# SowpatiLab/ribbit

Hardware: AMD Instinct MI355X
Metric: Gbases/s scanned (m=2..100) (higher is better)
Workload: dtype u32 bit planes

## Files before the change

ribbit_amd/csrc/kernels.hip:

```cpp
#include <hip/hip_runtime.h>

#include <algorithm>
#include <climits>
#include <type_traits>

#include "kernels.h"

namespace rb {

__device__ __forceinline__ uint32_t funnel(uint32_t hi, uint32_t lo, uint32_t sh) {
    return __builtin_amdgcn_alignbit(hi, lo, sh);
}

template <unsigned TT>
__device__ __forceinline__ uint32_t bitop3(uint32_t a, uint32_t b, uint32_t c) {
    return __builtin_amdgcn_bitop3_b32(a, b, c, TT);
}

__global__ __launch_bounds__(256) void pack_kernel(const uint8_t *__restrict__ ascii, int64_t length,
                                                   uint32_t *__restrict__ hi, uint32_t *__restrict__ lo,
                                                   uint32_t *__restrict__ brk, int64_t total_words,
                                                   uint32_t *__restrict__ zero_words, int n_zero) {
    const int64_t t = (int64_t)blockIdx.x * blockDim.x + threadIdx.x;
    if (blockIdx.x == 0)
// ... 43 lines not shown
            h |= __builtin_amdgcn_udot4(b2 & ok, weights, 0u, false) << (4 * i);
            l |= __builtin_amdgcn_udot4(lo1 & ok, weights, 0u, false) << (4 * i);
            b |= __builtin_amdgcn_udot4(bad, weights, 0u, false) << (4 * i);
        }
        if (left < 32) b |= 0xffffffffu << (uint32_t)left;
    }
    hi[t] = h; lo[t] = l; brk[t] = b;
}

void launch_pack(const uint8_t *dev_ascii, int64_t length, uint32_t *hi, uint32_t *lo, uint32_t *brk,
                 int64_t total_words, uint32_t *zero_words, int n_zero, hipStream_t stream) {
    const int threads = 256;
    const int64_t blocks = (total_words + threads - 1) / threads;
    hipLaunchKernelGGL(pack_kernel, dim3((unsigned)blocks), dim3(threads), 0, stream, dev_ascii, length, hi, lo, brk,
                       total_words, zero_words, n_zero);
}

constexpr int EV_STAGE = 256;

__device__ __forceinline__ int wave_inclusive_scan(int v) {
    v += __builtin_amdgcn_update_dpp(0, v, 0x111, 0xf, 0xf, true);
    v += __builtin_amdgcn_update_dpp(0, v, 0x112, 0xf, 0xf, true);
    v += __builtin_amdgcn_update_dpp(0, v, 0x114, 0xf, 0xf, true);
    v += __builtin_amdgcn_update_dpp(0, v, 0x118, 0xf, 0xf, true);
    v += __builtin_amdgcn_update_dpp(0, v, 0x142, 0xa, 0xf, false);
    v += __builtin_amdgcn_update_dpp(0, v, 0x143, 0xc, 0xf, false);
    return v;
}

struct EventSink {
    uint64_t *events;
    uint32_t *counters;
    uint32_t region_cap;
    uint32_t shard;
};

__device__ __forceinline__ void sink_flush(const EventSink &sk, volatile uint64_t *stage, int &staged, int lane) {
    if (staged == 0) return;
    uint32_t base = 0;
    if (lane == 0) base = atomicAdd(&sk.counters[sk.shard * EV_COUNTER_STRIDE], (uint32_t)staged);
    base = (uint32_t)__builtin_amdgcn_readfirstlane((int)base);
    uint64_t *dst = sk.events + (size_t)sk.shard * sk.region_cap;
    for (int i = lane; i < staged; i += 64) {
        const uint32_t idx = base + (uint32_t)i;
        if (idx < sk.region_cap) dst[idx] = stage[i];
    }
    __builtin_amdgcn_wave_barrier();
    staged = 0;
}

template <typename EndKind>
__device__ __forceinline__ void stage_events(const uint32_t (&S)[WORDS_PER_LANE], const uint32_t (&E)[WORDS_PER_LANE],
                                             uint32_t word0, uint32_t mlen, const EventSink &sink,
                                             volatile uint64_t *stage, int &staged, int lane, EndKind end_kind) {
    uint32_t Sv[WORDS_PER_LANE], Ev[WORDS_PER_LANE];
#pragma unroll
    for (int k = 0; k < WORDS_PER_LANE; k++) {
        Sv[k] = S[k]; Ev[k] = E[k];
        asm volatile("" : "+v"(Sv[k]), "+v"(Ev[k]));
    }
    int cnt = 0;
#pragma unroll
    for (int k = 0; k < WORDS_PER_LANE; k++) cnt += __popc(Sv[k]) + __popc(Ev[k]);
    const int incl = wave_inclusive_scan(cnt);
    const int total = __builtin_amdgcn_readlane(incl, 63);
    if (staged + total > EV_STAGE) sink_flush(sink, stage, staged, lane);
    const bool direct = total > EV_STAGE;
    uint32_t idx = (uint32_t)(incl - cnt);
    uint64_t *gdst = nullptr;
    if (direct) {
        uint32_t base = 0;
        if (lane == 0) base = atomicAdd(&sink.counters[sink.shard * EV_COUNTER_STRIDE], (uint32_t)total);
        idx += (uint32_t)__builtin_amdgcn_readfirstlane((int)base);
        gdst = sink.events + (size_t)sink.shard * sink.region_cap;
    } else {
        idx += (uint32_t)staged;
    }
#pragma unroll
    for (int k = 0; k < WORDS_PER_LANE; k++) {
        uint32_t both = Sv[k] | Ev[k];
        while (both) {
            const uint32_t b = (uint32_t)__builtin_ctz(both);
            both &= both - 1u;
            const uint32_t pos = ((word0 + (uint32_t)k) << 5) + b;
            const uint32_t kind = ((Sv[k] >> b) & 1u) ? (uint32_t)EV_START : end_kind(k, b, pos);
            const uint64_t e = ev_pack(pos, mlen, kind);
            if (direct) { if (idx < sink.region_cap) gdst[idx] = e; }
            else stage[idx] = e;
            idx++;
        }
    }
    if (!direct) staged += total;
    __builtin_amdgcn_wave_barrier();
}

constexpr int K = WORDS_PER_LANE;

#ifndef RB_COOP_MAX_LANES
#define RB_COOP_MAX_LANES 16
#endif
constexpr int COOP_SRC = 16;
struct CoopScratch { uint32_t w[COOP_SRC][20]; };

__device__ __forceinline__ void stage_events_coop(const uint32_t (&S)[WORDS_PER_LANE], const uint32_t (&E)[WORDS_PER_LANE], uint32_t word0, uint32_t mlen,
                                                  uint32_t brk_at, const uint32_t *s_brk, uint32_t length, CoopScratch &sc, const EventSink &sink,
                                                  volatile uint64_t *stage, int &staged, int lane) {
    uint32_t Sv[WORDS_PER_LANE], Ev[WORDS_PER_LANE];
#pragma unroll
    for (int k = 0; k < WORDS_PER_LANE; k++) {
        Sv[k] = S[k]; Ev[k] = E[k];
        asm volatile("" : "+v"(Sv[k]), "+v"(Ev[k]));
    }
    int cnt = 0;
#pragma unroll
    for (int k = 0; k < WORDS_PER_LANE; k++) cnt += __popc(Sv[k] | Ev[k]);
    const int incl = wave_inclusive_scan(cnt);
    const int total = __builtin_amdgcn_readlane(incl, 63);
    if (staged + total > EV_STAGE) sink_flush(sink, stage, staged, lane);
    const bool direct = total > EV_STAGE;
    uint32_t first = (uint32_t)(incl - cnt);
    uint64_t *gdst = nullptr;
    if (direct) {
        uint32_t base = 0;
        if (lane == 0) base = atomicAdd(&sink.counters[sink.shard * EV_COUNTER_STRIDE], (uint32_t)total);
        first += (uint32_t)__builtin_amdgcn_readfirstlane((int)base);
        gdst = sink.events + (size_t)sink.shard * sink.region_cap;
    } else {
        first += (uint32_t)staged;
    }
    unsigned long long todo = __ballot(cnt != 0);
    const int r = lane >> 2, j = lane & 3;
    do {
        const int rank = (int)__builtin_amdgcn_mbcnt_hi((uint32_t)(todo >> 32), __builtin_amdgcn_mbcnt_lo((uint32_t)todo, 0u));
        const bool mine = ((todo >> lane) & 1ull) != 0ull && rank < COOP_SRC;
        if (mine) {
            uint32_t *row = sc.w[rank];
#pragma unroll
            for (int k = 0; k < WORDS_PER_LANE; k++) { row[k] = Sv[k]; row[WORDS_PER_LANE + k] = Ev[k]; }
            row[16] = word0; row[17] = mlen; row[18] = brk_at; row[19] = first;
        }
        const unsigned long long handled = __ballot(mine);
        const int nsrc = __popcll(handled);
        todo &= ~handled;
        __builtin_amdgcn_wave_barrier();
        uint32_t s0 = 0, s1 = 0, e0 = 0, e1 = 0;
        if (r < nsrc) { s0 = sc.w[r][2 * j]; s1 = sc.w[r][2 * j + 1]; e0 = sc.w[r][WORDS_PER_LANE + 2 * j]; e1 = sc.w[r][WORDS_PER_LANE + 2 * j + 1]; }
        const int c = __popc(s0 | e0) + __popc(s1 | e1);
        const int q0 = __builtin_amdgcn_update_dpp(0, c, 0x00, 0xf, 0xf, true);
        const int q1 = __builtin_amdgcn_update_dpp(0, c, 0x55, 0xf, 0xf, true);
        const int q2 = __builtin_amdgcn_update_dpp(0, c, 0xaa, 0xf, 0xf, true);
        if (c != 0) {
            const uint32_t w0 = sc.w[r][16], ml = sc.w[r][17], bb = sc.w[r][18];
            uint32_t idx = sc.w[r][19] + (uint32_t)((j > 0 ? q0 : 0) + (j > 1 ? q1 : 0) + (j > 2 ? q2 : 0));
            auto expand = [&](uint32_t sw, uint32_t ew, uint32_t k) {
                uint32_t both = sw | ew;
                while (both) {
                    const uint32_t b = (uint32_t)__builtin_ctz(both);
                    both &= both - 1u;
                    const uint32_t pos = ((w0 + k) << 5) + b;
                    uint32_t kind = (uint32_t)EV_START;
                    if (!((sw >> b) & 1u))
                        kind = pos >= length ? (uint32_t)EV_END_EOS : (((s_brk[bb + k] >> b) & 1u) ? (uint32_t)EV_END_N : (uint32_t)EV_END_ZERO);
                    const uint64_t e = ev_pack(pos, ml, kind);
                    if (direct) { if (idx < sink.region_cap) gdst[idx] = e; }
                    else stage[idx] = e;
                    idx++;
                }
            };
            expand(s0, e0, 2u * (uint32_t)j);
            expand(s1, e1, 2u * (uint32_t)j + 1u);
        }
        __builtin_amdgcn_wave_barrier();
    } while (RB_COOP_MAX_LANES > COOP_SRC && todo != 0ull);
    if (!direct) staged += total;
}
__device__ __forceinline__ void group_filter(const uint32_t (&PASS)[K + 2], const uint32_t (&EVAL)[K + 2], int tj, uint32_t (&SV)[K + 1],
                                             uint32_t (&DR)[K]) {
    uint32_t J[K + 2], W[K + 2];
#pragma unroll
    for (int j = K + 1; j >= 1; j--) J[j] = PASS[j] | funnel(PASS[j], PASS[j - 1], 31);
    J[0] = PASS[0] | (PASS[0] << 1);
#pragma unroll
    for (int j = K + 1; j >= 1; j--) J[j] = J[j] | funnel(J[j], J[j - 1], 30);
    J[0] = J[0] | (J[0] << 2);
#pragma unroll
    for (int j = K + 1; j >= 1; j--) J[j] = J[j] | funnel(J[j], J[j - 1], 28);
    J[0] = J[0] | (J[0] << 4);
#pragma unroll
    for (int j = 0; j < K + 1; j++) J[j] = J[j] & funnel(J[j + 1], J[j], 1);
    J[K + 1] = J[K + 1] & (J[K + 1] >> 1);
#pragma unroll
    for (int j = 0; j < K + 1; j++) J[j] = J[j] & funnel(J[j + 1], J[j], 2);
    J[K + 1] = J[K + 1] & (J[K + 1] >> 2);
#pragma unroll
    for (int j = 0; j < K + 1; j++) J[j] = J[j] & funnel(J[j + 1], J[j], 4);
    J[K + 1] = J[K + 1] & (J[K + 1] >> 4);
#pragma unroll
    for (int j = 0; j < K + 2; j++) J[j] |= PASS[j];
#pragma unroll
    for (int j = 0; j < K + 2; j++) W[j] = J[j];
    {
        int span = 1;
#pragma unroll
        for (int step = 0; step < 4; step++) {
            const int sh = min(span, tj - span);
            if (sh > 0) {
#pragma unroll
                for (int j = 0; j < K + 1; j++) W[j] = W[j] & funnel(W[j + 1], W[j], (uint32_t)sh);
                W[K + 1] = W[K + 1] & (W[K + 1] >> sh);
                span += sh;
            }
        }
        span = 1;
#pragma unroll
        for (int step = 0; step < 4; step++) {
            const int sh = min(span, tj - span);
            if (sh > 0) {
#pragma unroll
                for (int j = K + 1; j >= 1; j--) W[j] = W[j] | funnel(W[j], W[j - 1], (uint32_t)(32 - sh));
                W[0] = W[0] | (W[0] << sh);
                span += sh;
            }
        }
    }
    auto special_ends = [&](int j) {
        const uint32_t jprev = j > 0 ? funnel(J[j], J[j - 1], 31) : (J[0] << 1);
        const uint32_t ev8 = j < K + 1 ? funnel(EVAL[j + 1], EVAL[j], 8) : (EVAL[K + 1] >> 8);
        const uint32_t g = ~J[j] & jprev & ~(EVAL[j] & ev8);
        return j == 0 ? 0u : (j == K + 1 ? (g & 0x0000ffffu) : g);
    };
    uint32_t special = 0;
#pragma unroll
    for (int j = 1; j < K + 2; j++) special |= special_ends(j);
    if (__ballot(special != 0) != 0ull) {
        uint32_t G[K + 2], JL[K + 2];
#pragma unroll
        for (int j = 0; j < K + 2; j++) { JL[j] = J[j]; G[j] = special_ends(j); }
#pragma unroll
        for (int j = 0; j < K + 1; j++) G[j] = funnel(G[j + 1], G[j], 1) & J[j];
        G[K + 1] = (G[K + 1] >> 1) & J[K + 1];
#pragma unroll
        for (int sh = 1; sh <= 8; sh <<= 1) {
#pragma unroll
            for (int j = 0; j < K + 1; j++) G[j] |= funnel(G[j + 1], G[j], (uint32_t)sh) & JL[j];
            G[K + 1] |= (G[K + 1] >> sh) & JL[K + 1];
#pragma unroll
            for (int j = 0; j < K + 1; j++) JL[j] = JL[j] & funnel(JL[j + 1], JL[j], (uint32_t)sh);
            JL[K + 1] = JL[K + 1] & (JL[K + 1] >> sh);
        }
#pragma unroll
        for (int j = 0; j < K + 1; j++) W[j] |= G[j];
    }
#pragma unroll
    for (int j = 0; j < K + 1; j++) SV[j] = W[j];
#pragma unroll
    for (int k = 0; k < K; k++) {
        const uint32_t jprev = funnel(J[k + 1], J[k], 31);
        const uint32_t svprev = funnel(W[k + 1], W[k], 31);
        DR[k] = ~J[k + 1] & jprev & ~svprev;
    }
}

constexpr int LDS_EXTRA = 40;

template <bool UNIFORM>
__device__ __forceinline__ uint32_t perfect_edges(const uint32_t (&Z)[K + 2], uint32_t t3, uint32_t t4, uint32_t t5,
                                                  uint32_t back, uint32_t (&SQ)[K], uint32_t (&EQ)[K]) {
    uint32_t D[K + 2];
#pragma unroll
    for (int j = 0; j < K + 1; j++) D[j] = Z[j] | funnel(Z[j + 1], Z[j], 1);
    D[K + 1] = Z[K + 1] | (Z[K + 1] >> 1);
#pragma unroll
    for (int j = 0; j < K + 1; j++) D[j] = D[j] | funnel(D[j + 1], D[j], 2);
    D[K + 1] = D[K + 1] | (D[K + 1] >> 2);
#pragma unroll
    for (int j = 0; j < K + 1; j++) D[j] = D[j] | funnel(D[j + 1], D[j], t3);
    D[K + 1] = D[K + 1] | (D[K + 1] >> t3);
#pragma unroll
    for (int j = 0; j < K + 1; j++) D[j] = D[j] | funnel(D[j + 1], D[j], t4);
    if (!UNIFORM || t5) {
        D[K + 1] = D[K + 1] | (D[K + 1] >> t4);
#pragma unroll
        for (int j = 0; j < K + 1; j++) D[j] = D[j] | funnel(D[j + 1], D[j], t5);
    }
    uint32_t any = 0;
#pragma unroll
    for (int k = 0; k < K; k++) {
        const int j = k + 1;
        const uint32_t prev_z = funnel(Z[j], Z[j - 1], 31);
        const uint32_t d_back = funnel(D[j], D[j - 1], back);
        SQ[k] = prev_z & ~D[j];
        EQ[k] = Z[j] & ~d_back;
        any = bitop3<0xFE>(SQ[k], EQ[k], any);
    }
    return any;
}

constexpr int CAND_CAP = 64;
#ifndef RB_CAND_DIRECT
#define RB_CAND_DIRECT 32
#endif
constexpr int CAND_DIRECT = RB_CAND_DIRECT;
struct CandQueue {
    uint32_t z[K + 2][CAND_CAP];
    uint32_t tag[CAND_CAP];
};

#ifndef RB_PERFECT_WAVES
#define RB_PERFECT_WAVES 4
#endif
__global__ __launch_bounds__(256) __attribute__((amdgpu_waves_per_eu(RB_PERFECT_WAVES, RB_PERFECT_WAVES))) void scan_perfect_kernel(DevicePlanes pl, PerfectLaunch pp, int motifs_per_block,
                                                           uint64_t *__restrict__ events,
                                                           uint32_t *__restrict__ counters) {
    __shared__ uint32_t s_hi[TILE_WORDS + LDS_EXTRA];
    __shared__ uint32_t s_lo[TILE_WORDS + LDS_EXTRA];
    __shared__ uint32_t s_brk[TILE_WORDS + 8];
    __shared__ uint64_t s_stage[4][EV_STAGE];
    __shared__ CandQueue s_cand[4];
    __shared__ CoopScratch s_coop[4];

    const int lane = threadIdx.x & 63;
    const int wave = __builtin_amdgcn_readfirstlane((int)(threadIdx.x >> 6));
    const int64_t tile_base = (int64_t)blockIdx.x * TILE_WORDS;

    const int bm_lo = pp.m_lo + (int)blockIdx.y * motifs_per_block;
    const int bm_hi = min(pp.m_hi, bm_lo + motifs_per_block - 1);
    const int q_hi = bm_hi >> 5;

    const int n_ext = TILE_WORDS + 4 + q_hi;
    for (int i = threadIdx.x; i < n_ext; i += 256) {
        s_hi[i] = pl.hi[tile_base - 1 + i];
        s_lo[i] = pl.lo[tile_base - 1 + i];
    }
    for (int i = threadIdx.x; i < TILE_WORDS + 2; i += 256) s_brk[i] = pl.brk[tile_base - 1 + i];
    __syncthreads();

    const int wm_lo = bm_lo + wave;
    const int wm_hi = bm_hi;
    if (wm_lo > wm_hi) return;

    const int lb = lane * K;
    uint32_t H[K + 2], Lo[K + 2], Bk[K + 2];
#pragma unroll
    for (int j = 0; j < K + 2; j++) { H[j] = s_hi[lb + j]; Lo[j] = s_lo[lb + j]; Bk[j] = s_brk[lb + j]; }

    uint32_t Hq[K + 3], Lq[K + 3];
    int cur_q = -1;
    const uint32_t length = (uint32_t)pl.length;
    const uint32_t word0 = (uint32_t)(tile_base + lb);

    EventSink sink;
    sink.events = events;
    sink.counters = counters;
    sink.region_cap = pp.ev_cap / EV_SHARDS;
    sink.shard = (blockIdx.x * 4u + (uint32_t)wave + blockIdx.y) % EV_SHARDS;
    volatile uint64_t *stage = s_stage[wave];
    int staged = 0;

    CandQueue &cq = s_cand[wave];
    int queued = 0;
    auto flush_candidates = [&]() {
        if (queued == 0) return;
        const bool live = lane < queued;
        const uint32_t tag = live ? cq.tag[lane] : 0u;
        const uint32_t src = tag & 0xffu, qm = tag >> 8;
        uint32_t Zq[K + 2];
#pragma unroll
        for (int j = 0; j < K + 2; j++) Zq[j] = live ? cq.z[j][lane] : 0xffffffffu;
        const int c1 = (qm <= 6u) ? 12 - (int)qm : (int)qm;
        const int sp = live ? min(c1, 32) : 32;
        const uint32_t t3 = (uint32_t)min(4, sp - 4);
        const uint32_t t4 = (uint32_t)min(8, sp - 4 - (int)t3);
        const uint32_t t5 = (uint32_t)(sp - 4) - t3 - t4;
        uint32_t SQ[K], EQ[K];
        uint32_t any = perfect_edges<false>(Zq, t3, t4, t5, 32u - (uint32_t)sp, SQ, EQ);
        if (!live) {
            any = 0;
#pragma unroll
            for (int k = 0; k < K; k++) { SQ[k] = 0; EQ[k] = 0; }
        }
#ifdef RB_ABLATE_STAGING
        const unsigned long long with_events = __ballot(any == 0xdeadbeefu);
#else
        const unsigned long long with_events = __ballot(any != 0);
#endif
        if (with_events != 0ull) {
            const uint32_t src_word0 = (uint32_t)tile_base + src * (uint32_t)K;
            if (__popcll(with_events) <= RB_COOP_MAX_LANES)
                stage_events_coop(SQ, EQ, src_word0, qm, src * (uint32_t)K + 1u, s_brk, length, s_coop[wave], sink, stage, staged, lane);
            else
                stage_events(SQ, EQ, src_word0, qm, sink, stage, staged, lane, [&](int k, uint32_t b, uint32_t pos) {
                    if (pos >= length) return (uint32_t)EV_END_EOS;
                    return ((s_brk[src * (uint32_t)K + (uint32_t)k + 1u] >> b) & 1u) ? (uint32_t)EV_END_N : (uint32_t)EV_END_ZERO;
                });
        }
        queued = 0;
        __builtin_amdgcn_wave_barrier();
    };

    for (int m = wm_lo; m <= wm_hi; m += 4) {
        const int q = m >> 5;
        const uint32_t r = (uint32_t)m & 31u;
        if (q != cur_q) {
            cur_q = q;
#pragma unroll
            for (int j = 0; j < K + 3; j++) { Hq[j] = s_hi[lb + j + q]; Lq[j] = s_lo[lb + j + q]; }
        }
        const int c1 = (m <= 6) ? 12 - m : m;
        const int sp = min(c1, 32);
        const uint32_t t3 = (uint32_t)min(4, sp - 4);
        const uint32_t t4 = (uint32_t)min(8, sp - 4 - (int)t3);
        const uint32_t t5 = (uint32_t)(sp - 4) - t3 - t4;

        uint32_t Z[K + 2];
#pragma unroll
        for (int j = 0; j < K + 2; j++) {
            const uint32_t hs = funnel(Hq[j + 1], Hq[j], r);
            const uint32_t ls = funnel(Lq[j + 1], Lq[j], r);
            Z[j] = bitop3<0xF6>(bitop3<0xBE>(H[j], hs, Bk[j]), Lo[j], ls);
        }
        if (sp >= 7) {
            bool cand;
            if (sp >= 31) {
                typedef unsigned short half2 __attribute__((ext_vector_type(2)));
                auto pk_min = [](uint32_t a, uint32_t b) {
                    const half2 m = __builtin_elementwise_min(__builtin_bit_cast(half2, a), __builtin_bit_cast(half2, b));
                    return __builtin_bit_cast(uint32_t, m);
                };
                uint32_t lowest = Z[0];
#pragma unroll
                for (int j = 1; j < K + 2; j++) lowest = pk_min(lowest, Z[j]);
                cand = (((lowest - 0x00010001u) & ~lowest) & 0x80008000u) != 0;
            } else {
                const uint32_t ones = sp >= 15 ? 0x01010101u : 0x11111111u;
                const uint32_t tops = sp >= 15 ? 0x80808080u : 0x88888888u;
                uint32_t hit = 0;
#pragma unroll
                for (int j = 0; j < K + 2; j++) hit = bitop3<0xBA>(Z[j] - ones, Z[j], hit);
                cand = (hit & tops) != 0;
            }
#ifdef RB_ABLATE_CHAIN
            const unsigned long long mask = __ballot(cand && Z[0] == 0xdeadbeefu);
#else
            const unsigned long long mask = __ballot(cand);
#endif
            if (mask == 0ull) continue;
            const int n = __popcll(mask);
            if (n <= CAND_DIRECT) {
                if (queued + n > CAND_CAP) flush_candidates();
                if (cand) {
                    const int slot = queued + (int)__builtin_amdgcn_mbcnt_hi((uint32_t)(mask >> 32), __builtin_amdgcn_mbcnt_lo((uint32_t)mask, 0u));
#pragma unroll
                    for (int j = 0; j < K + 2; j++) cq.z[j][slot] = Z[j];
                    cq.tag[slot] = (uint32_t)lane | ((uint32_t)m << 8);
                }
                queued += n;
                __builtin_amdgcn_wave_barrier();
                continue;
            }
        }
        uint32_t SQ[K], EQ[K];
        const uint32_t any = perfect_edges<true>(Z, t3, t4, t5, 32u - (uint32_t)sp, SQ, EQ);
#ifdef RB_ABLATE_STAGING
        const unsigned long long with_events = __ballot(any == 0xdeadbeefu);
#else
        const unsigned long long with_events = __ballot(any != 0);
#endif
        if (with_events != 0ull) {
            if (__popcll(with_events) <= RB_COOP_MAX_LANES)
                stage_events_coop(SQ, EQ, word0, (uint32_t)m, (uint32_t)lb + 1u, s_brk, length, s_coop[wave], sink, stage, staged, lane);
            else
                stage_events(SQ, EQ, word0, (uint32_t)m, sink, stage, staged, lane, [&](int k, uint32_t b, uint32_t pos) {
                    if (pos >= length) return (uint32_t)EV_END_EOS;
                    return ((Bk[k + 1] >> b) & 1u) ? (uint32_t)EV_END_N : (uint32_t)EV_END_ZERO;
                });
        }
    }
    flush_candidates();
    sink_flush(sink, stage, staged, lane);
}

static ScanSplit scan_split(const PerfectLaunch &pp, int nm, int64_t want_y, int max_y) {
    int motifs_per_block;
    if (pp.motifs_per_block > 0) {
        motifs_per_block = std::min(pp.motifs_per_block, nm);
    } else {
        const int gy = (int)(want_y < 1 ? 1 : (want_y > max_y ? max_y : want_y));
        motifs_per_block = (nm + gy - 1) / gy;
    }
    ScanSplit sp;
    sp.motifs_per_block = motifs_per_block;
    sp.grid_y = (nm + motifs_per_block - 1) / motifs_per_block;
    return sp;
}

ScanSplit launch_scan_perfect(const DevicePlanes &pl, const PerfectLaunch &pp, uint64_t *events, uint32_t *counters,
                              hipStream_t stream) {
    const int nm = pp.m_hi - pp.m_lo + 1;
    if (nm <= 0 || pl.ntiles <= 0) return {};
    const ScanSplit sp = scan_split(pp, nm, (2048 + pl.ntiles - 1) / pl.ntiles, (nm + 3) / 4);
    dim3 grid((unsigned)pl.ntiles, (unsigned)sp.grid_y);
    hipLaunchKernelGGL(scan_perfect_kernel, grid, dim3(256), 0, stream, pl, pp, sp.motifs_per_block, events, counters);
    return sp;
}

template <int ALLOWED>
__global__ __launch_bounds__(256) void scan_window_kernel(DevicePlanes pl, PerfectLaunch pp, int motifs_per_block,
                                                          uint64_t *__restrict__ events,
                                                          uint32_t *__restrict__ counters) {
    __shared__ uint32_t s_hi[TILE_WORDS + LDS_EXTRA];
    __shared__ uint32_t s_lo[TILE_WORDS + LDS_EXTRA];
    __shared__ uint32_t s_brk[TILE_WORDS + 8];
    __shared__ uint64_t s_stage[4][EV_STAGE];

    const int lane = threadIdx.x & 63;
    const int wave = __builtin_amdgcn_readfirstlane((int)(threadIdx.x >> 6));
    const int64_t tile_base = (int64_t)blockIdx.x * TILE_WORDS;

    const int bm_lo = pp.m_lo + (int)blockIdx.y * motifs_per_block;
    const int bm_hi = min(pp.m_hi, bm_lo + motifs_per_block - 1);
    const int q_hi = bm_hi >> 5;
    const int n_ext = TILE_WORDS + 4 + q_hi;
    for (int i = threadIdx.x; i < n_ext; i += 256) {
        s_hi[i] = pl.hi[tile_base - 1 + i];
        s_lo[i] = pl.lo[tile_base - 1 + i];
    }
    for (int i = threadIdx.x; i < TILE_WORDS + 2; i += 256) s_brk[i] = pl.brk[tile_base - 1 + i];
    __syncthreads();

    const int wm_lo = bm_lo + wave;
    const int wm_hi = bm_hi;
    if (wm_lo > wm_hi) return;

    const int lb = lane * K;
    uint32_t H[K + 2], Lo[K + 2];
    uint32_t EVAL[K + 1];
    {
        uint32_t B[K + 2];
#pragma unroll
        for (int j = 0; j < K + 2; j++) { H[j] = s_hi[lb + j]; Lo[j] = s_lo[lb + j]; B[j] = s_brk[lb + j]; }
#pragma unroll
        for (int j = 0; j < K + 1; j++) B[j] |= funnel(B[j + 1], B[j], 1);
        B[K + 1] |= B[K + 1] >> 1;
#pragma unroll
        for (int j = 0; j < K + 1; j++) B[j] |= funnel(B[j + 1], B[j], 2);
        B[K + 1] |= B[K + 1] >> 2;
#pragma unroll
        for (int j = 0; j < K + 1; j++) EVAL[j] = ~(B[j] | funnel(B[j + 1], B[j], 4));
    }

    uint32_t Hq[K + 3], Lq[K + 3];
    int cur_q = -1;
    const uint32_t length = (uint32_t)pl.length;
    const uint32_t word0 = (uint32_t)(tile_base + lb);

    EventSink sink;
    sink.events = events;
    sink.counters = counters;
    sink.region_cap = pp.ev_cap / EV_SHARDS;
    sink.shard = (blockIdx.x * 4u + (uint32_t)wave + blockIdx.y) % EV_SHARDS;
    volatile uint64_t *stage = s_stage[wave];
    int staged = 0;

    for (int m = wm_lo; m <= wm_hi; m += 4) {
        const int q = m >> 5;
        const uint32_t r = (uint32_t)m & 31u;
        if (q != cur_q) {
            cur_q = q;
#pragma unroll
            for (int j = 0; j < K + 3; j++) { Hq[j] = s_hi[lb + j + q]; Lq[j] = s_lo[lb + j + q]; }
        }
        uint32_t A1[K + 2], B1[K + 2], C1[K + 2];
#pragma unroll
        for (int j = 0; j < K + 2; j++) {
            const uint32_t hs = funnel(Hq[j + 1], Hq[j], r);
            const uint32_t ls = funnel(Lq[j + 1], Lq[j], r);
            A1[j] = (H[j] ^ hs) | (Lo[j] ^ ls);
        }
#pragma unroll
        for (int j = 0; j < K + 2; j++) {
            const uint32_t sa = (j <= K) ? funnel(A1[j + 1 <= K + 1 ? j + 1 : j], A1[j], 1) : (A1[j] >> 1);
            B1[j] = A1[j] & sa;
            A1[j] = A1[j] | sa;
        }
#pragma unroll
        for (int j = 0; j < K + 2; j++) {
            const uint32_t sa = (j <= K) ? funnel(A1[j + 1 <= K + 1 ? j + 1 : j], A1[j], 2) : (A1[j] >> 2);
            const uint32_t sb = (j <= K) ? funnel(B1[j + 1 <= K + 1 ? j + 1 : j], B1[j], 2) : (B1[j] >> 2);
            if (ALLOWED == 2) C1[j] = (B1[j] & sa) | (A1[j] & sb);
            B1[j] = B1[j] | sb | (A1[j] & sa);
            A1[j] = A1[j] | sa;
        }
        uint32_t PASS[K + 1];
#pragma unroll
        for (int j = 0; j < K + 1; j++) {
            const uint32_t sa = funnel(A1[j + 1], A1[j], 4);
            const uint32_t sb = funnel(B1[j + 1], B1[j], 4);
            uint32_t bad;
            if (ALLOWED == 2) {
                const uint32_t sc = funnel(C1[j + 1], C1[j], 4);
                bad = C1[j] | sc | (B1[j] & sa) | (A1[j] & sb);
            } else {
                bad = B1[j] | sb | (A1[j] & sa);
            }
            PASS[j] = EVAL[j] & ~bad;
        }
        uint32_t ST[K], EN[K];
        uint32_t any = 0;
#pragma unroll
        for (int k = 0; k < K; k++) {
            const uint32_t prev = funnel(PASS[k + 1], PASS[k], 31);
            ST[k] = PASS[k + 1] & ~prev;
            EN[k] = ~PASS[k + 1] & prev;
            any |= ST[k] | EN[k];
        }
        if (__ballot(any != 0) != 0ull) {
            stage_events(ST, EN, word0, (uint32_t)m, sink, stage, staged, lane, [&](int k, uint32_t b, uint32_t pos) {
                if ((EVAL[k + 1] >> b) & 1u) return (uint32_t)EV_END_ZERO;
                return (pos + 7u >= length) ? (uint32_t)EV_END_EOS : (uint32_t)EV_END_N;
            });
        }
    }
    sink_flush(sink, stage, staged, lane);
}

ScanSplit launch_scan_window(const DevicePlanes &pl, const PerfectLaunch &pp, int allowed_mismatches, uint64_t *events,
                             uint32_t *counters, hipStream_t stream) {
    const int nm = pp.m_hi - pp.m_lo + 1;
    if (nm <= 0 || pl.ntiles <= 0) return {};
    const ScanSplit sp = scan_split(pp, nm, (2048 + pl.ntiles - 1) / pl.ntiles, (nm + 3) / 4);
    dim3 grid((unsigned)pl.ntiles, (unsigned)sp.grid_y);
    if (allowed_mismatches == 1)
        hipLaunchKernelGGL(scan_window_kernel<1>, grid, dim3(256), 0, stream, pl, pp, sp.motifs_per_block, events, counters);
    else
        hipLaunchKernelGGL(scan_window_kernel<2>, grid, dim3(256), 0, stream, pl, pp, sp.motifs_per_block, events, counters);
    return sp;
}

constexpr int RUN_SAT = 1 << 20;

__global__ __launch_bounds__(256) __attribute__((amdgpu_waves_per_eu(2, 4))) void scan_anchored_kernel(DevicePlanes pl, PerfectLaunch pp, int motifs_per_block, int hl,
                                                            uint32_t *__restrict__ xa, int64_t xa_stride) {
    __shared__ uint32_t s_hi[64 * K + LDS_EXTRA];
    __shared__ uint32_t s_lo[64 * K + LDS_EXTRA];

    const int lane = threadIdx.x & 63;
    const int wave = __builtin_amdgcn_readfirstlane((int)(threadIdx.x >> 6));
    const int64_t tile_base = (int64_t)blockIdx.x * anchored_tile_words(hl);
    const int64_t first = tile_base - (int64_t)hl * K - 1;

    const int bm_lo = pp.m_lo + (int)blockIdx.y * motifs_per_block;
    const int bm_hi = min(pp.m_hi, bm_lo + motifs_per_block - 1);
    const int q_hi = (bm_hi + 2) >> 5;
    const int n_ext = 64 * K + 4 + q_hi;
    for (int i = threadIdx.x; i < n_ext; i += 256) {
        s_hi[i] = pl.hi[first + i];
        s_lo[i] = pl.lo[first + i];
    }
    __syncthreads();

    const int nmb = bm_hi - bm_lo + 1;
    const int per = (nmb + 3) >> 2;
    const int wm_lo = bm_lo + wave * per;
    const int wm_hi = min(bm_hi, wm_lo + per - 1);
    if (wm_lo > wm_hi) return;

    const int lb = lane * K;
    const bool own_lane = lane >= hl && lane < 64 - hl;
    uint32_t H[K + 2], Lo[K + 2];
#pragma unroll
    for (int j = 0; j < K + 2; j++) { H[j] = s_hi[lb + j]; Lo[j] = s_lo[lb + j]; }

    const int64_t w_own0 = tile_base + (int64_t)(lane - hl) * K;
    const int64_t length = pl.length;
    const int64_t lane_lo = (w_own0 - 1) * 32, lane_hi = (w_own0 + K + 1) * 32;
    const bool edge_lane = lane_lo < 0 || lane_hi > length - (int64_t)(wm_hi + 2);
    const bool edge_wave = __ballot(edge_lane) != 0ull;

    uint32_t Hq[K + 3], Lq[K + 3];
    int cur_q = -1;

    uint32_t AN[5][K + 2];
#pragma unroll
    for (int a = 0; a < 5; a++)
#pragma unroll
        for (int j = 0; j < K + 2; j++) AN[a][j] = 0;

    const int s_first = max(1, wm_lo - 2);
    const int s_last = wm_hi + 2;
    auto step = [&](auto slot_c, int s) {
        constexpr int R = decltype(slot_c)::value;
        constexpr int R1 = (R + 4) % 5, R3 = (R + 2) % 5, R4 = (R + 1) % 5;
        const int q = s >> 5;
        const uint32_t r = (uint32_t)s & 31u;
        if (q != cur_q) {
            cur_q = q;
#pragma unroll
            for (int j = 0; j < K + 3; j++) { Hq[j] = s_hi[lb + j + q]; Lq[j] = s_lo[lb + j + q]; }
        }
        uint32_t X[K];
#pragma unroll
        for (int k = 0; k < K; k++) {
            const uint32_t hs = funnel(Hq[k + 2], Hq[k + 1], r);
            const uint32_t ls = funnel(Lq[k + 2], Lq[k + 1], r);
            X[k] = ~((H[k + 1] ^ hs) | (Lo[k + 1] ^ ls));
        }
        if (edge_wave) {
#pragma unroll
            for (int k = 0; k < K; k++) {
                const int64_t bp = (w_own0 + k) * 32;
                const int64_t f = (length - s) - bp;
                const uint32_t force = f <= 0 ? 0xffffffffu : (f >= 32 ? 0u : (0xffffffffu << (uint32_t)f));
                X[k] = (bp < 0) ? 0u : (X[k] | force);
            }
        }
        const int two_s = 2 * s;
        int lead1[K], trail1[K];
        int span_lead = 0, span_trail = 0;
        bool alive = true;
#pragma unroll
        for (int k = 0; k < K; k++) {
            const uint32_t nx = ~X[k];
            lead1[k] = nx ? __builtin_ctz(nx) : 32;
            trail1[k] = nx ? __builtin_clz(nx) : 32;
            span_lead += alive ? lead1[k] : 0;
            alive = alive && (nx == 0u);
        }
        const bool span_full = alive;
        alive = true;
#pragma unroll
        for (int k = K - 1; k >= 0; k--) {
            span_trail += alive ? trail1[k] : 0;
            alive = alive && (X[k] == 0xffffffffu);
        }
        int accL = span_trail, accR = span_lead, fullL = span_full ? 1 : 0, fullR = fullL;
        for (int d = 1; d < hl; d <<= 1) {
            int a2 = __shfl_up(accL, d), f2 = __shfl_up(fullL, d);
            if (lane < d) { a2 = 0; f2 = 0; }
            accL = min(accL + (fullL ? a2 : 0), RUN_SAT);
            fullL &= f2;
            a2 = __shfl_down(accR, d); f2 = __shfl_down(fullR, d);
            if (lane + d > 63) { a2 = 0; f2 = 0; }
            accR = min(accR + (fullR ? a2 : 0), RUN_SAT);
            fullR &= f2;
        }
        int left_in = __shfl_up(accL, 1);
        int right_in = __shfl_down(accR, 1);
        if (lane == 0) left_in = 0;
        if (lane == 63) right_in = 0;
        int CL[K], CR[K];
        {
            int c = left_in;
#pragma unroll
            for (int k = 0; k < K; k++) { CL[k] = c; c = (X[k] == 0xffffffffu) ? min(c + 32, RUN_SAT) : trail1[k]; }
            c = right_in;
#pragma unroll
            for (int k = K - 1; k >= 0; k--) { CR[k] = c; c = (X[k] == 0xffffffffu) ? min(c + 32, RUN_SAT) : lead1[k]; }
        }
#pragma unroll
        for (int k = 0; k < K; k++) {
            const uint32_t x = X[k];
            const bool isfull = x == 0xffffffffu;
// ... 656 lines not shown
```

Before: 435.2.

## Prefilter long motifs on hi plane only and recompute candidate Z from LDS

For periods of 31 and above, the candidate prefilter now builds Z from the hi bit plane and break mask only. The lo-plane term is added only when a wave falls back to the full edge path. The candidate queue no longer stores the K+2 Z words per candidate; the flush step rebuilds Z from the shared tiles using the tag's lane and motif. For short periods the lo plane now reuses the already loaded unshifted Lo registers plus one extra word instead of reloading Lq. This cuts per-iteration ALU, register and LDS-store work, but the hi-only filter is looser and may queue more false candidates, and each flush does extra LDS reads.

```diff
diff --git a/ribbit_amd/csrc/kernels.hip b/ribbit_amd/csrc/kernels.hip
--- a/ribbit_amd/csrc/kernels.hip
+++ b/ribbit_amd/csrc/kernels.hip
@@ -369,7 +369,6 @@
 #endif
 constexpr int CAND_DIRECT = RB_CAND_DIRECT;
 struct CandQueue {
-    uint32_t z[K + 2][CAND_CAP];
     uint32_t tag[CAND_CAP];
 };
 
@@ -411,7 +410,12 @@
 #pragma unroll
     for (int j = 0; j < K + 2; j++) { H[j] = s_hi[lb + j]; Lo[j] = s_lo[lb + j]; Bk[j] = s_brk[lb + j]; }
 
-    uint32_t Hq[K + 3], Lq[K + 3];
+    uint32_t Hq[K + 3];
+#ifdef RB_PREFILTER_FULLZ
+    uint32_t Lq[K + 3];
+#else
+    const uint32_t lo_next = s_lo[lb + K + 2];
+#endif
     int cur_q = -1;
     const uint32_t length = (uint32_t)pl.length;
     const uint32_t word0 = (uint32_t)(tile_base + lb);
@@ -431,9 +435,18 @@
         const bool live = lane < queued;
         const uint32_t tag = live ? cq.tag[lane] : 0u;
         const uint32_t src = tag & 0xffu, qm = tag >> 8;
+        const uint32_t sb = src * (uint32_t)K, sq = sb + (qm >> 5), sr = qm & 31u;
         uint32_t Zq[K + 2];
-#pragma unroll
-        for (int j = 0; j < K + 2; j++) Zq[j] = live ? cq.z[j][lane] : 0xffffffffu;
+        {
+            uint32_t h0 = s_hi[sq], l0 = s_lo[sq];
+#pragma unroll
+            for (int j = 0; j < K + 2; j++) {
+                const uint32_t h1 = s_hi[sq + j + 1], l1 = s_lo[sq + j + 1];
+                const uint32_t z = bitop3<0xF6>(bitop3<0xBE>(s_hi[sb + j], funnel(h1, h0, sr), s_brk[sb + j]), s_lo[sb + j], funnel(l1, l0, sr));
+                Zq[j] = live ? z : 0xffffffffu;
+                h0 = h1; l0 = l1;
+            }
+        }
         const int c1 = (qm <= 6u) ? 12 - (int)qm : (int)qm;
         const int sp = live ? min(c1, 32) : 32;
         const uint32_t t3 = (uint32_t)min(4, sp - 4);
@@ -471,7 +484,11 @@
         if (q != cur_q) {
             cur_q = q;
 #pragma unroll
-            for (int j = 0; j < K + 3; j++) { Hq[j] = s_hi[lb + j + q]; Lq[j] = s_lo[lb + j + q]; }
+            for (int j = 0; j < K + 3; j++) Hq[j] = s_hi[lb + j + q];
+#ifdef RB_PREFILTER_FULLZ
+#pragma unroll
+            for (int j = 0; j < K + 3; j++) Lq[j] = s_lo[lb + j + q];
+#endif
         }
         const int c1 = (m <= 6) ? 12 - m : m;
         const int sp = min(c1, 32);
@@ -479,12 +496,24 @@
         const uint32_t t4 = (uint32_t)min(8, sp - 4 - (int)t3);
         const uint32_t t5 = (uint32_t)(sp - 4) - t3 - t4;
 
+#ifdef RB_PREFILTER_FULLZ
+        const bool h_only = false;
+        auto lq = [&](int j) { return Lq[j]; };
+#else
+        const bool h_only = sp >= 31;
+        auto lq = [&](int j) { return j < K + 2 ? Lo[j] : lo_next; };
+#endif
         uint32_t Z[K + 2];
-#pragma unroll
-        for (int j = 0; j < K + 2; j++) {
-            const uint32_t hs = funnel(Hq[j + 1], Hq[j], r);
-            const uint32_t ls = funnel(Lq[j + 1], Lq[j], r);
-            Z[j] = bitop3<0xF6>(bitop3<0xBE>(H[j], hs, Bk[j]), Lo[j], ls);
+        if (h_only) {
+#pragma unroll
+            for (int j = 0; j < K + 2; j++) Z[j] = bitop3<0xBE>(H[j], funnel(Hq[j + 1], Hq[j], r), Bk[j]);
+        } else {
+#pragma unroll
+            for (int j = 0; j < K + 2; j++) {
+                const uint32_t hs = funnel(Hq[j + 1], Hq[j], r);
+                const uint32_t ls = funnel(lq(j + 1), lq(j), r);
+                Z[j] = bitop3<0xF6>(bitop3<0xBE>(H[j], hs, Bk[j]), Lo[j], ls);
+            }
         }
         if (sp >= 7) {
             bool cand;
@@ -517,14 +546,23 @@
                 if (queued + n > CAND_CAP) flush_candidates();
                 if (cand) {
                     const int slot = queued + (int)__builtin_amdgcn_mbcnt_hi((uint32_t)(mask >> 32), __builtin_amdgcn_mbcnt_lo((uint32_t)mask, 0u));
-#pragma unroll
-                    for (int j = 0; j < K + 2; j++) cq.z[j][slot] = Z[j];
                     cq.tag[slot] = (uint32_t)lane | ((uint32_t)m << 8);
                 }
                 queued += n;
                 __builtin_amdgcn_wave_barrier();
                 continue;
             }
+#ifndef RB_PREFILTER_FULLZ
+            if (h_only) {
+                uint32_t l0 = s_lo[lb + q];
+#pragma unroll
+                for (int j = 0; j < K + 2; j++) {
+                    const uint32_t l1 = s_lo[lb + j + 1 + q];
+                    Z[j] = bitop3<0xF6>(Z[j], Lo[j], funnel(l1, l0, r));
+                    l0 = l1;
+                }
+            }
+#endif
         }
         uint32_t SQ[K], EQ[K];
         const uint32_t any = perfect_edges<true>(Z, t3, t4, t5, 32u - (uint32_t)sp, SQ, EQ);
```

Result: no change. 431.4 (-0.9%).
